# Rouslan/NTracer

Measured on AMD Instinct MI355X. Metric: Mrays/s (primary+shadow), 6-D hypercube @1920x1080, higher is better.
Workload: dtype f32

## Files before the change

ntracer_amd/csrc/nt_box.hpp:

```cpp
#pragma once
#include <type_traits>
#include "nt_pixel.hpp"
#include "nt_box_span.hpp"

namespace {

__device__ __forceinline__ bool box_may_hit(int n, const float *dots, float sx, float sy, float sq) {
    const float osq = dots[0];
    const float ov = fmaf(-dots[2], sy, fmaf(dots[1], sx, dots[3]));
    const float rad2 = (float)n * (1.0f + NT_FUZZ) * (1.0f + NT_FUZZ) * 1.001f;
#ifdef NT_EXP_SKIP_SLABS
    return false;
#else
    return !((osq - rad2) * sq > ov * ov * 1.0001f);
#endif
}

__device__ __forceinline__ void box_background(float in, float &r, float &g, float &b) {
    if (in > 0.0f) { r = in; g = in; b = in; }
    else { r = 0.0f; g = -in; b = -in; }
}

template <int N>
__device__ __forceinline__ void box_color(const float (&o)[N], const float (&dir)[N], bool maybe, float &r, float &g, float &b) {
    bool done = false;
    float shade = 0.0f;

    {
        float num[N];
        bool pre[N];
        float aK = 0.0f, bK = 1.0f, oK = 0.0f;
        bool any = false;
#pragma unroll
        for (int i = 0; i < N; ++i) {
            const float di = dir[i];
            const float s = di < 0.0f ? 1.0f : -1.0f;
            num[i] = s - o[i];
            pre[i] = maybe && ((num[i] > 0.0f && di > 0.0f) || (num[i] < 0.0f && di < 0.0f));
            const float a = fabsf(num[i]), bb = fabsf(di);
            if (pre[i] && (!any || a * bK > aK * bb)) { aK = a; bK = bb; oK = o[i]; any = true; }
        }
        const float mu = 1e-4f * (1.0f + fabsf(oK));
        const float aKm = (aK - mu) * (1.0f - 1e-6f);
#pragma unroll
        for (int i = 0; i < N; ++i) {
            const bool tie = pre[i] && !done && !(fabsf(num[i]) * bK < fabsf(dir[i]) * aKm);
            if (__builtin_amdgcn_ballot_w64(tie) != 0ull) {
                const float di = dir[i];
                const float dist = num[i] / di;
                bool ok = tie && dist > 0.0f;
#pragma unroll
                for (int j = 0; j < N; ++j) {
                    if (j != i) {
                        const float p = dir[j] * dist + o[j];
                        ok = ok && !(fabsf(p) > (1.0f + NT_FUZZ));
                    }
                }
                if (ok) {
                    done = true;
                    if (dist >= FLT_MAX) shade = -1.0f;
                    else {
                        const float sine = di * (di < 0.0f ? 1.0f : -1.0f);
                        shade = sine <= 0.0f ? -sine : 0.0f;
                    }
                }
            }
        }
    }
    if (done && shade >= 0.0f) {
        r = shade * 1.0f;
        g = shade * 0.5f;
        b = shade * 0.5f;
    } else {
        box_background(dir[0], r, g, b);
    }
}

#ifndef NT_BOX_INLINE_MAX_N
#define NT_BOX_INLINE_MAX_N 8
#endif
#ifndef NT_BOX_SETS_MAX_N
#define NT_BOX_SETS_MAX_N NT_BOX_INLINE_MAX_N
#endif
template <int N>
__device__ __forceinline__ void box_classify(const float (&o)[N], const float (&v)[N], float m, bool maybe, bool &hit, bool &unclear,
                                             float &x, float (&near)[N], float &tn, float &vK) {
    float tn2 = -INFINITY;
    tn = -INFINITY;
    vK = 0.0f;
    float tnp = -INFINITY, tfp = INFINITY;
    const float m1p = 1.0f + m;
#pragma unroll
    for (int j = 0; j < N; ++j) {
        const float inv = __builtin_amdgcn_rcpf(v[j]);
        const float c0 = -o[j] * inv;
        const float nr = c0 - fabsf(inv);
        near[j] = nr;
        tnp = fmaxf(tnp, fmaf(-fabsf(inv), m1p, c0));
        tfp = fminf(tfp, fmaf(fabsf(inv), m1p, c0));
        const bool later = nr > tn;
        tn2 = __builtin_amdgcn_fmed3f(tn, tn2, nr);
        vK = later ? v[j] : vK;
        tn = fmaxf(tn, nr);
    }
    const bool miss = tnp > tfp || tfp < 0.0f;
    const float c = 1.0f - m;
    float sum = 0.0f;
#pragma unroll
    for (int j = 0; j < N; ++j) sum = sum + fmaxf(fabsf(fmaf(v[j], tn, o[j])), c);
    const bool inside = sum - (float)N * c <= 1.5f * m;
    const bool sole = (tn - tn2) * fabsf(vK) > m;
    const bool front = tn > 1e-3f && tn < 1e30f;
    hit = maybe && !miss && inside && sole && front;
    unclear = maybe && !miss && !hit;
#ifdef NT_EXP_NOUNCLEAR
    unclear = false;
#endif
    x = hit ? vK : v[0];
}

__device__ __forceinline__ float nt_vmax(float a, float b) { float r; asm("v_max_f32 %0, %1, %2" : "=v"(r) : "v"(a), "v"(b)); return r; }
__device__ __forceinline__ float nt_vmin(float a, float b) { float r; asm("v_min_f32 %0, %1, %2" : "=v"(r) : "v"(a), "v"(b)); return r; }
__device__ __forceinline__ float nt_vmax3(float a, float b, float c) { float r; asm("v_max3_f32 %0, %1, %2, %3" : "=v"(r) : "v"(a), "v"(b), "v"(c)); return r; }
__device__ __forceinline__ float nt_vmin3(float a, float b, float c) { float r; asm("v_min3_f32 %0, %1, %2, %3" : "=v"(r) : "v"(a), "v"(b), "v"(c)); return r; }
__device__ __forceinline__ float nt_vmed3(float a, float b, float c) { float r; asm("v_med3_f32 %0, %1, %2, %3" : "=v"(r) : "v"(a), "v"(b), "v"(c)); return r; }
__device__ __forceinline__ float nt_vmax_abs(float a, float b) { float r; asm("v_max_f32 %0, |%1|, %2" : "=v"(r) : "v"(a), "v"(b)); return r; }
__device__ __forceinline__ float nt_vmax3_abs(float a, float b, float c) { float r; asm("v_max3_f32 %0, %1, |%2|, |%3|" : "=v"(r) : "v"(a), "v"(b), "v"(c)); return r; }
__device__ __forceinline__ float nt_vmin_abs(float a, float b) { float r; asm("v_min_f32 %0, |%1|, %2" : "=v"(r) : "v"(a), "v"(b)); return r; }

#ifndef NT_BOX_TIE_SHORTCUT
#define NT_BOX_TIE_SHORTCUT 1
#endif
#ifndef NT_BOX_TIE_SHORTCUT_MIN_N
#define NT_BOX_TIE_SHORTCUT_MIN_N 6
#endif
#ifndef NT_BOX_TIE_SHORTCUT_MAX_N
#define NT_BOX_TIE_SHORTCUT_MAX_N 8
#endif
#ifndef NT_BOX_TIE_SURE_MAX_ORIGIN
#define NT_BOX_TIE_SURE_MAX_ORIGIN 4.5f
#endif
#ifndef NT_BOX_TIE_SHORTCUT_MIN_WAVES
#define NT_BOX_TIE_SHORTCUT_MIN_WAVES 32768
#endif
#define NT_BOX_SETS_SURE 0x01000000u
#ifndef NT_BOX_STRIP_SPAN
#define NT_BOX_STRIP_SPAN 1
#endif
template <int N>
constexpr bool nt_box_tie_shortcut() { return NT_BOX_TIE_SHORTCUT != 0 && N >= NT_BOX_TIE_SHORTCUT_MIN_N && N <= NT_BOX_TIE_SHORTCUT_MAX_N && N <= NT_BOX_SETS_MAX_N; }

#ifndef NT_BOX_CLASSIFY_SETS_MIN_N
#define NT_BOX_CLASSIFY_SETS_MIN_N 6
#endif
#ifndef NT_BOX_CLASSIFY_SETS_MAX_N
#define NT_BOX_CLASSIFY_SETS_MAX_N 7
#endif
template <int N>
__device__ __forceinline__ void box_classify_sets(const float (&o)[N], const float (&v)[N], float m, uint32_t sets, bool &hit, bool &unclear,
                                                  float &x) {
    float tn = -INFINITY, tn2 = -INFINITY, vK = 0.0f;
    float tnp = -INFINITY, tfp = INFINITY;
    const float m1p = 1.0f + m;
#pragma unroll
    for (int j = 0; j < N; ++j) {
        if (((sets >> (10 + j)) & 1u) != 0u) {
            const float inv = __builtin_amdgcn_rcpf(v[j]);
            const float c0 = -o[j] * inv;
            tfp = nt_vmin(tfp, fmaf(fabsf(inv), m1p, c0));
            if (((sets >> j) & 1u) != 0u) {
                const float nr = c0 - fabsf(inv);
                tnp = nt_vmax(tnp, fmaf(-fabsf(inv), m1p, c0));
                const bool later = nr > tn;
                tn2 = nt_vmed3(tn, tn2, nr);
                vK = later ? v[j] : vK;
                tn = nt_vmax(tn, nr);
            }
        }
    }
    const bool miss = tnp > tfp || tfp < 0.0f;
    const float c = 1.0f - m;
    float sum = 0.0f;
#ifndef NT_EXP_SETS_MASKS
    asm volatile("" : "+s"(sets));
#endif
#pragma unroll
    for (int j = 0; j < N; ++j) {
        if (((sets >> (10 + j)) & 1u) != 0u) {
            asm volatile("" : "+v"(sum));
            sum = sum + nt_vmax_abs(fmaf(v[j], tn, o[j]), c);
        }
    }
    const bool inside = sum - (float)__builtin_popcount((sets >> 10) & 0x3ffu) * c <= 1.5f * m;
    const bool sole = (tn - tn2) * fabsf(vK) > m;
    const bool front = tn > 1e-3f && tn < 1e30f;
    hit = !miss && inside && sole && front;
    unclear = !miss && !hit;
    x = hit ? vK : v[0];
}

template <int N>
__device__ __forceinline__ void box_entries(const float (&o)[N], const float (&v)[N], float (&near)[N], float &tn, float &vK) {
    tn = -INFINITY;
    vK = 0.0f;
#pragma unroll
    for (int j = 0; j < N; ++j) {
        const float inv = __builtin_amdgcn_rcpf(v[j]);
        const float nr = fmaf(-o[j], inv, -fabsf(inv));
        near[j] = nr;
        vK = nr > tn ? v[j] : vK;
        tn = fmaxf(tn, nr);
    }
}

template <int N>
__device__ __forceinline__ void box_resolve(const float (&o)[N], const float (&v)[N], float len, float m, const float (&near)[N], float tn,
                                            float vK, bool unclear, bool &hit, float &x) {
    const float aK = fabsf(vK);
    const float slack = m * __builtin_amdgcn_rcpf(aK), lim = 1.0f - 0.5f * m;
    bool inT[N], inC[N];
    float d[N];
    uint32_t anyC = 0u;
#pragma unroll
    for (int j = 0; j < N; ++j) {
        const bool early = (tn - near[j]) * aK > m;
        const bool robust = fmaf(fabsf(v[j]), slack, fabsf(fmaf(v[j], tn, o[j]))) <= lim;
        inT[j] = unclear && !early;
        inC[j] = unclear && !(robust && early);
        d[j] = 0.0f;
        if (__builtin_amdgcn_ballot_w64(inC[j]) != 0ull) {
            d[j] = v[j] / len;
            anyC |= 1u << j;
        }
    }
    bool done = false, found = false;
    float xs = v[0];
#pragma unroll
    for (int i = 0; i < N; ++i) {
        const bool cand = inT[i] && !done;
        if (__builtin_amdgcn_ballot_w64(cand) != 0ull) {
            const float di = d[i];
            const float dist = ((di < 0.0f ? 1.0f : -1.0f) - o[i]) / di;
            bool ok = cand && di != 0.0f && dist > 0.0f;
#pragma unroll
            for (int j = 0; j < N; ++j) {
                if (j != i && ((anyC >> j) & 1u) != 0u) {
                    const float p = d[j] * dist + o[j];
                    ok = ok && !(inC[j] && fabsf(p) > (1.0f + NT_FUZZ));
                }
            }
            if (ok) {
                done = true;
                if (!(dist >= FLT_MAX)) { found = true; xs = v[i]; }
            }
        }
    }
    if (unclear) {
        hit = found;
        x = xs;
    }
}

typedef __attribute__((address_space(1))) uint8_t *nt_gptr;
__device__ __forceinline__ nt_gptr uniform_ptr(uint8_t *p) {
    const unsigned long long v = reinterpret_cast<unsigned long long>(p);
    const uint32_t lo = (uint32_t)__builtin_amdgcn_readfirstlane((int)(uint32_t)v), hi = (uint32_t)__builtin_amdgcn_readfirstlane((int)(uint32_t)(v >> 32));
    return (nt_gptr)(((unsigned long long)hi << 32) | lo);
}
#define NT_G32(p) (*(__attribute__((address_space(1))) uint32_t *)(p))

template <typename P>
__device__ __forceinline__ void emit_f32x3_at(const NtTarget &tg, P p, float r, float gb) {
    r = r > 0.0f ? r : 0.0f;
    r = r < 1.0f ? r : 1.0f;
    gb = gb > 0.0f ? gb : 0.0f;
    gb = gb < 1.0f ? gb : 1.0f;
    uint32_t vr = __float_as_uint(r), vgb = __float_as_uint(gb);
    uint3 w;
    if (tg.plain_f32[0] == 0 && tg.plain_f32[1] == 1 && tg.plain_f32[2] == 2 && !tg.reversed) {
        w.x = bswap32(vr);
        w.y = bswap32(vgb);
        w.z = w.y;
    } else {
        if (!tg.reversed) { vr = bswap32(vr); vgb = bswap32(vgb); }
        w.x = tg.plain_f32[tg.reversed ? 2 : 0] == 0 ? vr : vgb;
        w.y = tg.plain_f32[1] == 0 ? vr : vgb;
        w.z = tg.plain_f32[tg.reversed ? 0 : 2] == 0 ? vr : vgb;
    }
    if constexpr (std::is_same<P, nt_gptr>::value) {
        typedef uint32_t u32x3 __attribute__((ext_vector_type(3)));
        u32x3 v;
        v.x = w.x; v.y = w.y; v.z = w.z;
        *(__attribute__((address_space(1))) u32x3 *)(p) = v;
    } else {
        *reinterpret_cast<uint3 *>(p) = w;
    }
}
__device__ __forceinline__ void emit_f32x3(const NtTarget &tg, long long offset, float r, float gb) { emit_f32x3_at(tg, tg.dest + offset, r, gb); }

__device__ __forceinline__ float sqrt_in_range(float x) {
    const float s = __builtin_amdgcn_sqrtf(x);
    const float s_dn = __uint_as_float(__float_as_uint(s) - 1u), s_up = __uint_as_float(__float_as_uint(s) + 1u);
    const float vp = fmaf(-s_dn, s, x), vs = fmaf(-s_up, s, x);
    float r = vp <= 0.0f ? s_dn : s;
    r = vs > 0.0f ? s_up : r;
    return r;
}
__device__ __forceinline__ float sqrt_wave(float x) {
    if (__builtin_amdgcn_ballot_w64(!(x >= 0x1p-96f && x < 0x1p96f)) == 0ull) return sqrt_in_range(x);
    return sqrtf(x);
}

template <int N, bool PLAIN, bool DEFER = false, bool REDO = false, bool F32 = false, bool TIE = false>
__device__ __forceinline__ bool box_pixel(const NtTarget &tg, const PixelRef &pr, const float (&org)[N], float (&dir)[N], float sq,
                                          const float (&dots)[4], float sx, float sy, float margin, bool rowhit = true, int face = -1,
                                          uint32_t sets = 0u, bool noclass = false) {
    constexpr bool INL = (F32 || PLAIN) && !REDO && !DEFER;
    const bool redo = REDO || (INL && noclass);
    const bool maybe = redo || (rowhit && (DEFER || INL || box_may_hit(N, dots, sx, sy, sq)));
    float r, g, b;
    bool hit = false, unclear = false;
    float x = dir[0];
#ifndef NT_EXP_NOCLASSIFY
    float near[N], tn = 0.0f, vK = 0.0f;
    constexpr bool CSETS = INL && N >= NT_BOX_CLASSIFY_SETS_MIN_N && N <= NT_BOX_CLASSIFY_SETS_MAX_N;
    auto exact_on_sets = [&]() {
        const float len = sqrt_wave(sq);
        float d[N];
#pragma unroll
        for (int j = 0; j < N; ++j) {
            d[j] = 0.0f;
            if ((sets >> (10 + j)) & 1u) d[j] = dir[j] / len;
        }
        bool done = false;
        x = dir[0];
#pragma unroll
        for (int i = 0; i < N; ++i) {
// ... 307 lines not shown
    }
    if (!(tlo > thi)) {
        code = 15u;
#pragma unroll
        for (int j = 0; j < N; ++j) {
            const float nr = ((vc[j] < 0.0f ? 1.0f : -1.0f) - org[j]) * __builtin_amdgcn_rcpf(vc[j]);
            tn2 = nt_vmed3(tn, tn2, nr);
            const bool later = nr > tn;
            vK = later ? vc[j] : vK;
            gK = later ? g[j] : gK;
            oK = later ? org[j] : oK;
            K = later ? j : K;
            tn = nt_vmax(tn, nr);
        }
        const float vKa = vK - gK, vKb = vK + gK;
        if (K < 13 && vKa * vKb > 0.0f) {
            const float num = (vK < 0.0f ? 1.0f : -1.0f) - oK;
            const float t1 = num * __builtin_amdgcn_rcpf(vKa), t2 = num * __builtin_amdgcn_rcpf(vKb);
            const float t_lo = nt_vmin(t1, t2) * (1.0f - 1e-6f), t_hi = nt_vmax(t1, t2) * (1.0f + 1e-6f);
            const float rK = m * __builtin_amdgcn_rcpf(fabsf(vK) - gK) * (1.0f + 1e-6f);
            bool ok = t_lo > 1e-3f && t_hi < 1e30f;
#pragma unroll
            for (int j = 0; j < N; ++j) {
                const float va = vc[j] - g[j], vb = vc[j] + g[j];
                const float pmax = org[j] + nt_vmax(vb * t_lo, vb * t_hi);
                const float pmin = org[j] + nt_vmin(va * t_lo, va * t_hi);
                const float lim = (1.0f - m - 1e-4f) - (fabsf(vc[j]) + g[j]) * rK;
                ok = ok && (j == K || (pmax <= lim && pmin >= -lim));
            }
            if (ok) code = (uint32_t)K + 1u;
        }
        if (code == 15u && !((tn - tn2) * fabsf(vK) > m)) code = 14u;
        if (code >= 14u) {
            if (sets != nullptr && N <= 10) {
                auto range = [&](int j, float &A, float &B, float &vabs) {
                    const float va = vc[j] - g[j], vb = vc[j] + g[j];
                    const float num = (vc[j] < 0.0f ? 1.0f : -1.0f) - org[j];
                    const float e1 = num * __builtin_amdgcn_rcpf(va), e2 = num * __builtin_amdgcn_rcpf(vb);
                    const float lo = nt_vmin(e1, e2), hi = nt_vmax(e1, e2);
                    const bool same = va * vb > 0.0f;
                    A = same ? lo - fabsf(lo) * 1e-6f : -INFINITY;
                    B = same ? hi + fabsf(hi) * 1e-6f : INFINITY;
                    vabs = same ? fabsf(vc[j]) - g[j] : 0.0f;
                };
                float rA[N], rB[N], rV[N];
                float TN = -INFINITY, TH = -INFINITY;
#pragma unroll
                for (int j = 0; j < N; ++j) {
                    range(j, rA[j], rB[j], rV[j]);
                    TN = nt_vmax(TN, rA[j]);
                    TH = nt_vmax(TH, rB[j]);
                }
                float vmin = INFINITY;
#pragma unroll
                for (int j = 0; j < N; ++j) vmin = rB[j] >= TN ? nt_vmin(vmin, rV[j]) : vmin;
                const float M = m * __builtin_amdgcn_rcpf(vmin) * (1.0f + 1e-5f);
                uint32_t T = 0u, C = 0u;
                float t_lo = INFINITY;
                const float t_hi = TH;
#pragma unroll
                for (int j = 0; j < N; ++j) {
                    const bool inT = rB[j] >= TN - M;
                    T |= inT ? 1u << j : 0u;
                    t_lo = inT ? nt_vmin(t_lo, rA[j]) : t_lo;
                }
#pragma unroll
                for (int j = 0; j < N; ++j) {
                    const float va = vc[j] - g[j], vb = vc[j] + g[j];
                    const float pmax = org[j] + nt_vmax(vb * t_lo, vb * t_hi);
                    const float pmin = org[j] + nt_vmin(va * t_lo, va * t_hi);
                    const float lim = 1.0f - m - 1e-4f;
                    const bool inC = ((T >> j) & 1u) != 0u || !(pmax <= lim && pmin >= -lim);
                    C |= inC ? 1u << j : 0u;
                }
                const bool valid = vmin > 0.0f && t_lo > 1e-3f && t_hi < 1e30f;
                *sets = valid ? (0x80000000u | (C << 10) | T) : 0u;
                if constexpr (SURE) {
                    float wmax = 0.0f;
                    uint32_t far_axes = 0u;
#pragma unroll
                    for (int j = 0; j < N; ++j) {
                        wmax = nt_vmax3_abs(wmax, vc[j] - g[j], vc[j] + g[j]);
                        far_axes |= (__float_as_uint(org[j]) & 0x7fffffffu) > __float_as_uint(NT_BOX_TIE_SURE_MAX_ORIGIN) ? 1u << j : 0u;
                    }
                    const bool sure = valid && C == T && (T & far_axes) == 0u && (t_hi - t_lo) * wmax <= 1.0f;
                    *sets |= sure ? NT_BOX_SETS_SURE : 0u;
                }
            }
        }
    }
    return (unsigned long long)code | ((unsigned long long)sets_value << 32);
}
template <int N>
__device__ __forceinline__ uint32_t box_stretch_code(const float (&org)[N], const float (&right)[N], const float (&up)[N], const float (&fwd)[N],
                                                     const NtTarget &tg, int y, int col) {
    return (uint32_t)box_stretch_code2<N, false>(org, right, up, fwd, tg, y, col);
}

template <int N>
__global__ __launch_bounds__(256) void box_cull_kernel(NtCameraFixed cam, NtTarget tg, uint32_t *out, int ncols) {
    float org[N], right[N], up[N], fwd[N];
    load_camera<N>(cam, org, right, up, fwd);
    const int word = (int)blockIdx.x, row = (int)blockIdx.y * 8 + (int)(threadIdx.x >> 5);
    const int col = word * 32 + (int)(threadIdx.x & 31);
    uint32_t code = 0u;
    if (row < tg.row_count && col < ncols) {
        const int orow = tg.row_begin + row;
        const int y = nt_image_row(tg, orow);
        code = box_stretch_code<N>(org, right, up, fwd, tg, y, col);
    }
    uint32_t packed = code << (4 * (threadIdx.x & 7));
    packed |= (uint32_t)__shfl_xor((int)packed, 1, 64);
    packed |= (uint32_t)__shfl_xor((int)packed, 2, 64);
    packed |= (uint32_t)__shfl_xor((int)packed, 4, 64);
    if (row < tg.row_count && (threadIdx.x & 7) == 0) out[((size_t)blockIdx.z * tg.row_count + row) * tg.cull_words + (col >> 3)] = packed;
}

#ifdef NT_EXP_NOSTORE
#define NT_EXP_STORE_IF if (tg.width < 0)
#else
#define NT_EXP_STORE_IF
#endif
#ifndef NT_TILE_OCC
#define NT_TILE_OCC
#endif
#ifndef NT_BOX_PIN_UP
#define NT_BOX_PIN_UP 1
#endif
#ifndef NT_BOX_LEAN_GROUPS_MAX_N
#define NT_BOX_LEAN_GROUPS_MAX_N 20
#endif
__device__ __forceinline__ bool guard_clear(float t) { return fabsf(__builtin_amdgcn_fractf(t) - 0.5f) > fmaf(t, 0x1p-18f, 0x1p-18f); }
__device__ __forceinline__ float lean_quotient(float d, float sy, float uu, float m2bu, float bb) {
    return fabsf(d) * __builtin_amdgcn_rsqf(fmaf(sy, fmaf(sy, uu, m2bu), bb));
}
template <int N>
__device__ __forceinline__ void pick_component(uint32_t K, const float (&base)[N], const float (&upv)[N], float &bK, float &uK) {
    bK = base[0];
    uK = upv[0];
#pragma unroll
    for (int j = 1; j < N; ++j) {
        bK = K == (uint32_t)j ? base[j] : bK;
        uK = K == (uint32_t)j ? upv[j] : uK;
    }
}
template <int N>
__device__ __forceinline__ float row_dir(const float (&base)[N], const float (&upv)[N], float sy, float (&dir)[N]) {
#pragma unroll
    for (int j = 0; j < N; ++j) dir[j] = base[j] - upv[j] * sy;
    float sq = dir[0] * dir[0];
#pragma unroll
    for (int j = 1; j < N; ++j) sq = sq + dir[j] * dir[j];
    return sq;
}
#ifndef NT_BOX_PASS_ROWS
#define NT_BOX_PASS_ROWS 64
#endif
__device__ __forceinline__ int nt_low_bit(uint32_t m) { return __builtin_ctz(m); }
__device__ __forceinline__ int nt_low_bit(unsigned long long m) { return __builtin_ctzll(m); }
__device__ __forceinline__ int nt_count_bits(uint32_t m) { return __builtin_popcount(m); }
__device__ __forceinline__ int nt_count_bits(unsigned long long m) { return __builtin_popcountll(m); }
__device__ __forceinline__ void nt_clear_bit(uint32_t &m, int bit) { asm("s_bitset0_b32 %0, %1" : "+s"(m) : "s"(bit)); }
__device__ __forceinline__ void nt_clear_bit(unsigned long long &m, int bit) { asm("s_bitset0_b64 %0, %1" : "+s"(m) : "s"(bit)); }
__device__ __forceinline__ void nt_set_bit(uint32_t &m, int bit) { asm("s_bitset1_b32 %0, %1" : "+s"(m) : "s"(bit)); }
__device__ __forceinline__ void nt_set_bit(unsigned long long &m, int bit) { asm("s_bitset1_b64 %0, %1" : "+s"(m) : "s"(bit)); }
__device__ __forceinline__ void nt_drop_low_bit(uint32_t &m, int) { m &= m - 1u; }
__device__ __forceinline__ void nt_drop_low_bit(unsigned long long &m, int bit) { nt_clear_bit(m, bit); }
template <int N, bool F32, int ROWS, int WAVES, bool TIE = false>
__global__ __launch_bounds__(64 * WAVES) NT_TILE_OCC void box_tile_kernel(NtCameraFixed cam, NtTarget tg) {
    static_assert(!TIE || (!F32 && ROWS == 64 && nt_box_tie_shortcut<N>()), "the short cut: packed RGB, 64 x 1, the dimensions it is built for");
    static_assert(ROWS == 8 || ROWS == 16 || ROWS == 64, "a wave's rows: a qword of sixteen codes in LDS or fewer, or one row a lane");
    static_assert(WAVES >= 1 && WAVES <= 4 && WAVES * ROWS <= 64, "the codes of a tile are the work of one wave, a row per lane");
    static_assert(WAVES == 1 ? ROWS == 64 : ROWS <= 16, "one wave a block renders the 64 rows whose codes it worked out itself");
    constexpr int R = ROWS;
    constexpr bool REG = WAVES == 1;
    constexpr int LDS_N = REG ? 1 : 64;
    __shared__ uint32_t s_code[LDS_N];
    __shared__ unsigned long long s_rows[REG ? 1 : 4];
    constexpr bool ALLIN = F32 || N <= NT_BOX_INLINE_MAX_N;
    constexpr bool SETS_LDS = ALLIN && N <= NT_BOX_SETS_MAX_N;
    constexpr uint32_t SETS_MASK = 0x800fffffu | (TIE ? NT_BOX_SETS_SURE : 0u);
    __shared__ uint32_t s_sets[SETS_LDS ? LDS_N : 1];
    __shared__ int s_abort;
    uint32_t lane_cs = 0u;
    const int tid = (int)threadIdx.x;
    const int lane = tid & 63;
    const int wv = __builtin_amdgcn_readfirstlane(tid >> 6);
#ifdef NT_EXP_TRACE
    const unsigned long long trace_t0 = wall_clock64();
    unsigned trace_rows = 0u;
    unsigned long long trace_t1 = 0ull;
#endif
    const unsigned nframes = gridDim.z - (unsigned)tg.lead_frames;
    unsigned frame = blockIdx.z;
    if (tg.lead_frames > 0) {
        const unsigned cols = gridDim.x, q = cols / 4u;
        const bool middle = blockIdx.x >= q && blockIdx.x < cols - q;
        if (!middle) frame -= (unsigned)tg.lead_frames;
        if (frame >= nframes) return;
    }
    float org[N], right[N], up[N], fwd[N], dir[N];
    load_camera<N>(cam, frame, org, right, up, fwd);
    float margin = fabsf(org[0]);
#pragma unroll
    for (int j = 1; j < N; ++j) margin = fmaxf(margin, fabsf(org[j]));
    margin = NT_BOX_MARGIN * (1.0f + margin);
    float dots[4];
    if (cam.buf) {
        const float *dp = cam.dots + (size_t)frame * 4;
        dots[0] = dp[0]; dots[1] = dp[1]; dots[2] = dp[2]; dots[3] = dp[3];
    } else {
        dots[0] = cam.odots[0]; dots[1] = cam.odots[1]; dots[2] = cam.odots[2]; dots[3] = cam.odots[3];
    }
    const int tile_row0 = (int)blockIdx.y * WAVES * R;
    bool strip_out = false;
    if constexpr (NT_BOX_STRIP_SPAN != 0 && N <= NT_BOX_SPAN_MAX_N) {
      if (cam.span != nullptr) {
        const float *sp = cam.span + (size_t)frame * 2;
        const float span_lo = sp[0], span_hi = sp[1];
        const int x_first = (int)blockIdx.x * 64;
        const int x_last = x_first + 63 < tg.width ? x_first + 63 : tg.width - 1;
        const float sx_a = tg.fovI * ((float)x_first - tg.half_w), sx_b = tg.fovI * ((float)x_last - tg.half_w);
        strip_out = fmaxf(sx_a, sx_b) < span_lo || fminf(sx_a, sx_b) > span_hi;
      }
    }
    if (REG || wv == (int)((blockIdx.x + blockIdx.y + frame) % (unsigned)WAVES)) {
        if (tg.abort_word != nullptr) {
            const bool ab = nt_aborted(tg);
            if constexpr (REG) { if (ab) return; }
            else { if (lane == 0) s_abort = ab ? 1 : 0; }
        }
        uint32_t code = 0u;
        uint32_t row_sets = 0u;
        const int trow = tg.row_il > 0 ? ((int)blockIdx.y * WAVES + lane / R) + tg.row_il * (lane % R) : tile_row0 + lane;
        if (!strip_out && lane < WAVES * R && trow < tg.row_count) {
            const int orow = tg.row_begin + trow;
            const int y = nt_image_row(tg, orow);
            if (y < tg.height) {
                const unsigned long long cs = box_stretch_code2<N, (N <= NT_BOX_SETS_MAX_N), TIE>(org, right, up, fwd, tg, y, (int)blockIdx.x);
                code = (uint32_t)cs;
                row_sets = (uint32_t)(cs >> 32);
            }
        }
        if constexpr (REG) {
            lane_cs = (SETS_LDS ? row_sets & SETS_MASK : 0u) | (code << 20);
        } else {
            if (SETS_LDS) s_sets[lane] = row_sets;
            {
                const unsigned long long m0 = __builtin_amdgcn_ballot_w64(code == 0u), m1 = __builtin_amdgcn_ballot_w64(code >= 1u && code <= 13u),
                                         m2 = __builtin_amdgcn_ballot_w64(code == 15u), m3 = __builtin_amdgcn_ballot_w64(code == 14u);
                if (lane == 0) {
                    s_rows[0] = m0;
                    s_rows[1] = m1;
                    s_rows[2] = m2;
                    s_rows[3] = m3;
                }
            }
            uint32_t packed = code << (4 * (lane & 7));
            packed |= (uint32_t)__shfl_xor((int)packed, 1, 64);
            packed |= (uint32_t)__shfl_xor((int)packed, 2, 64);
            packed |= (uint32_t)__shfl_xor((int)packed, 4, 64);
            if ((lane & 7) == 0) {
                const int grp = lane >> 3;
                const int slot = R == 8 ? 2 * grp : grp;
                s_code[slot] = packed;
                if (R == 8) s_code[slot + 1] = 0u;
            }
        }
    }
    if constexpr (!REG) {
        __syncthreads();
        if (tg.abort_word != nullptr && s_abort != 0) return;
    }
#ifdef NT_EXP_TRACE
    trace_t1 = wall_clock64();
#endif
    constexpr int PASS = R == 64 ? NT_BOX_PASS_ROWS : R;
    static_assert(PASS == R || (R == 64 && PASS == 16), "NT_BOX_PASS_ROWS: 64 or 16");
    typedef typename std::conditional<PASS == 64, unsigned long long, uint32_t>::type mask_t;
    const int wrow0 = tile_row0 + wv * R;
    const int il = tg.row_il;
    const int wfirst = il > 0 ? (int)blockIdx.y * WAVES + wv : wrow0;
    if (wfirst < tg.row_count) {
        typedef uint32_t nt_u32x4 __attribute__((ext_vector_type(4)));
        typedef __attribute__((address_space(4))) const nt_u32x4 *nt_rowtab;
        typedef uint32_t nt_u32x16 __attribute__((ext_vector_type(16), aligned(16)));
        typedef __attribute__((address_space(4))) const nt_u32x16 *nt_rowtab4;
        constexpr bool GROUPS = !F32 && N <= NT_BOX_LEAN_GROUPS_MAX_N;
        uint8_t *const frame_base = tg.dest + (long long)frame * tg.frame_stride;
#define NT_ROW_LOAD(rr)                     \
        const nt_u32x4 row_e = tab[(rr)];   \
        const float sy = __uint_as_float(row_e.x)
#define NT_ROW_OFF() ((long long)(((unsigned long long)row_e.w << 32) | row_e.z) + (long long)frame * tg.frame_stride)
#define NT_ROW_PTR() uniform_ptr(frame_base + (long long)(((unsigned long long)row_e.w << 32) | row_e.z))
#define NT_GROUP_PTR(k) uniform_ptr(frame_base + (long long)(((unsigned long long)grp_e[4 * (k) + 3] << 32) | grp_e[4 * (k) + 2]))
#define NT_LANE_OFF() ({ asm volatile("" : "+v"(xoff)); xoff; })
#define NT_CLEAR_BIT(mask, bit) nt_clear_bit(mask, bit)
#define NT_SET_BIT(mask, bit) nt_set_bit(mask, bit)
        int x = (int)blockIdx.x * 64 + lane;
        x = x < tg.width ? x : tg.width - 1;
        uint32_t xoff = (uint32_t)x * (uint32_t)tg.bpp;
        const float sx = tg.fovI * ((float)x - tg.half_w);
        float base[N];
#pragma unroll
        for (int j = 0; j < N; ++j) base[j] = fwd[j] + right[j] * sx;
        float upv[N];
#pragma unroll
        for (int j = 0; j < N; ++j) {
            upv[j] = up[j];
            if (NT_BOX_PIN_UP || F32 || j == 0) asm volatile("" : "+v"(upv[j]));
        }
        float bb = 0.0f, bu = 0.0f, uu = 0.0f;
        bool fastsq = true;
        if (!F32) {
#pragma unroll
            for (int j = 0; j < N; ++j) {
                bb = fmaf(base[j], base[j], bb);
                bu = fmaf(base[j], up[j], bu);
                uu = fmaf(up[j], up[j], uu);
            }
            fastsq = __builtin_amdgcn_ballot_w64(!(bu * bu <= bb * uu * 0.0625f)) == 0ull;
        }
        const float maxv = (float)tg.plain_maxval;
        const float inv_maxv2 = 1.0f / (maxv * maxv);
        const float m2bu = (-2.0f * bu) * inv_maxv2;
        bb = bb * inv_maxv2;
        uu = uu * inv_maxv2;
        const uint32_t lane_code = (lane_cs >> 20) & 15u;
        unsigned long long rows_culled, rows_face, rows_rays, rows_tie;
        if constexpr (REG) {
            rows_culled = __builtin_amdgcn_ballot_w64(lane_code == 0u);
            rows_face = __builtin_amdgcn_ballot_w64(lane_code >= 1u && lane_code <= 13u);
            rows_rays = __builtin_amdgcn_ballot_w64(lane_code == 15u);
            rows_tie = __builtin_amdgcn_ballot_w64(lane_code == 14u);
        } else {
            auto rows_of = [&](int k) {
                const unsigned long long m = s_rows[k];
                return (((unsigned long long)(uint32_t)__builtin_amdgcn_readfirstlane((int)(uint32_t)(m >> 32)) << 32) |
                        (uint32_t)__builtin_amdgcn_readfirstlane((int)(uint32_t)m)) >> (wv * R);
            };
            rows_culled = rows_of(0);
            rows_face = rows_of(1);
            rows_rays = rows_of(2);
            rows_tie = rows_of(3);
        }
        const int lrow = il > 0 ? wfirst + il * lane : wrow0 + lane;
        const int ly = nt_image_row(tg, tg.row_begin + lrow);
        const unsigned long long rows_valid = __builtin_amdgcn_ballot_w64(lane < R && lrow < tg.row_count && ly < tg.height);
#pragma unroll 1
        for (int pass = 0; pass < R / PASS; ++pass) {
        const int slot0 = PASS * pass;
        const int row0 = wrow0 + slot0;
        const int hfirst = il > 0 ? wfirst + il * slot0 : row0;
        if (hfirst >= tg.row_count) break;
        mask_t redo_bits = 0u;
        unsigned long long rowcodes = 0ull;
        if constexpr (!REG) {
            rowcodes = ((unsigned long long)(uint32_t)__builtin_amdgcn_readfirstlane((int)s_code[2 * wv + 1]) << 32) |
                       (uint32_t)__builtin_amdgcn_readfirstlane((int)s_code[2 * wv]);
        }
        auto slot_word = [&](int rr) { return (uint32_t)__builtin_amdgcn_readlane((int)lane_cs, slot0 + rr); };
        auto code_of = [&](int rr) {
            if constexpr (REG) return (slot_word(rr) >> 20) & 15u;
            else return (uint32_t)(rowcodes >> (4 * rr)) & 15u;
        };
        auto sets_of = [&](int rr) {
            if constexpr (!SETS_LDS) return 0u;
            else if constexpr (REG) return slot_word(rr) & SETS_MASK;
            else return (uint32_t)__builtin_amdgcn_readfirstlane((int)s_sets[wv * R + rr]);
        };
        auto rows_with_code = [&](uint32_t c) {
            if constexpr (REG) return (mask_t)(__builtin_amdgcn_ballot_w64(lane_code == c) >> slot0);
            else return (mask_t)__builtin_amdgcn_ballot_w64(lane < PASS && ((uint32_t)(rowcodes >> (4 * (lane & 15))) & 15u) == c);
        };
        const mask_t valid = R > PASS ? (mask_t)(rows_valid >> slot0) & (mask_t)((1ull << (PASS & 63)) - 1ull) : (mask_t)rows_valid;
        const nt_rowtab tab = (nt_rowtab)tg.rowtab + (il > 0 ? row0 : tg.row_begin + row0);
        mask_t quick = (mask_t)(rows_culled >> slot0) & valid, inner = (mask_t)(rows_face >> slot0) & valid;
        mask_t todo = (mask_t)((ALLIN ? rows_rays | rows_tie : rows_rays) >> slot0) & valid;
        if (!ALLIN) redo_bits = (mask_t)(rows_tie >> slot0) & valid;
#ifdef NT_EXP_TRACE
        trace_rows += (unsigned)nt_count_bits(quick) | ((unsigned)nt_count_bits(inner) << 8) |
                      ((unsigned)nt_count_bits((mask_t)(rows_rays >> slot0) & valid) << 16) |
                      ((unsigned)nt_count_bits((mask_t)(rows_tie >> slot0) & valid) << 24);
#endif
        if (!F32) {
            if (!fastsq) {
                todo |= quick | inner;
                quick = 0u;
                inner = 0u;
            }
            auto lean_rows = [&](auto sel8) {
            constexpr bool SEL8 = decltype(sel8)::value;
#ifdef NT_EXP_RED_BY_SHIFT
#define NT_RED_OF(q, d0) ((q) & (uint32_t)((int32_t)__float_as_uint(d0) >> 31))
#else
#define NT_RED_OF(q, d0) ((d0) > 0.0f ? (q) : 0u)
#endif
            auto put_quick = [&](nt_gptr out, float t, float d0) {
                if (SEL8) {
                    const uint32_t q = __float_as_uint(t + 8388608.0f);
                    NT_EXP_STORE_IF NT_G32(out) = __builtin_amdgcn_perm(NT_RED_OF(q, d0), q, tg.plain_sel);
                    return;
                }
                uint32_t q = (uint32_t)(t + 0.5f);
                q = q < tg.plain_maxval ? q : tg.plain_maxval;
                const uint32_t w = NT_RED_OF(q, d0) * tg.plain_mul[0] + q * (tg.plain_mul[1] + tg.plain_mul[2]);
                NT_EXP_STORE_IF NT_G32(out) = tg.reversed ? w : bswap32(w);
            };
            auto put_face = [&](nt_gptr out, float t, float th) {
                if (SEL8) {
                    NT_EXP_STORE_IF NT_G32(out) = __builtin_amdgcn_perm(__float_as_uint(t + 8388608.0f), __float_as_uint(th + 8388608.0f), tg.plain_sel);
                    return;
                }
                uint32_t qr = (uint32_t)(t + 0.5f), qgb = (uint32_t)(th + 0.5f);
                qr = qr < tg.plain_maxval ? qr : tg.plain_maxval;
                qgb = qgb < tg.plain_maxval ? qgb : tg.plain_maxval;
                const uint32_t w = qr * tg.plain_mul[0] + qgb * (tg.plain_mul[1] + tg.plain_mul[2]);
                NT_EXP_STORE_IF NT_G32(out) = tg.reversed ? w : bswap32(w);
            };
            auto full_groups = [](mask_t mask) { return mask & (mask >> 1) & (mask >> 2) & (mask >> 3) & (mask_t)(PASS == 64 ? 0x1111111111111111ull : 0x1111ull); };
            auto lean_group = [&](int g, auto row, auto put) {
                const nt_u32x16 grp_e = *(nt_rowtab4)(tab + g);
                float a[4], b[4];
                unsigned long long fail[4];
#pragma unroll
                for (int k = 0; k < 4; ++k) fail[k] = __builtin_amdgcn_ballot_w64(!row(__uint_as_float(grp_e[4 * k]), a[k], b[k]));
                if (__builtin_expect(((fail[0] | fail[1]) | (fail[2] | fail[3])) == 0ull, 1)) {
                    const uint32_t xo = NT_LANE_OFF();
                    put(NT_GROUP_PTR(0) + xo, a[0], b[0]);
                    put(NT_GROUP_PTR(1) + xo, a[1], b[1]);
                    put(NT_GROUP_PTR(2) + xo, a[2], b[2]);
                    put(NT_GROUP_PTR(3) + xo, a[3], b[3]);
                } else {
                    todo |= (mask_t)((fail[0] != 0ull ? 1u : 0u) | (fail[1] != 0ull ? 2u : 0u) | (fail[2] != 0ull ? 4u : 0u) | (fail[3] != 0ull ? 8u : 0u)) << g;
#pragma unroll
                    for (int k = 0; k < 4; ++k) {
                        if (fail[k] == 0ull) {
                            uint32_t xo = xoff;
                            asm volatile("" : "+v"(xo));
                            put(NT_GROUP_PTR(k) + xo, a[k], b[k]);
                        }
                    }
                }
            };
            auto culled_row = [&](float sy, float &t, float &d0) {
#ifdef NT_EXP_RED_BY_SHIFT
                d0 = upv[0] * sy - base[0];
#else
                d0 = base[0] - upv[0] * sy;
#endif
                t = lean_quotient(d0, sy, uu, m2bu, bb);
                return guard_clear(t);
            };
            auto face_row = [&](float bK, float uK, float sy, float &t, float &th) {
                const float dK = bK - uK * sy;
                t = lean_quotient(dK, sy, uu, m2bu, bb);
                th = t * 0.5f;
                return guard_clear(t) && guard_clear(th);
            };
            if (GROUPS) {
                mask_t full = full_groups(quick);
                quick &= ~(full * 15u);
                while (full != 0u) {
                    const int g = nt_low_bit(full);
                    NT_CLEAR_BIT(full, g);
                    lean_group(g, culled_row, put_quick);
                }
            }
            mask_t quick_stored = 0u;
            for (mask_t rest = quick; rest != 0u;) {
                const int rr = nt_low_bit(rest);
                NT_CLEAR_BIT(rest, rr);
                NT_ROW_LOAD(rr);
                float t, d0;
                if (__builtin_expect(__builtin_amdgcn_ballot_w64(!culled_row(sy, t, d0)) == 0ull, 1)) {
                    put_quick(NT_ROW_PTR() + NT_LANE_OFF(), t, d0);
                    NT_SET_BIT(quick_stored, rr);
                }
            }
            todo |= quick & ~quick_stored;
            while (inner != 0u) {
                const uint32_t code0 = code_of(nt_low_bit(inner));
                float bK0, uK0;
                pick_component<N>(code0 - 1u, base, upv, bK0, uK0);
                mask_t same = inner & rows_with_code(code0);
                inner &= ~same;
                if (GROUPS) {
                    mask_t full = full_groups(same);
                    same &= ~(full * 15u);
                    while (full != 0u) {
                        const int g = nt_low_bit(full);
                        NT_CLEAR_BIT(full, g);
                        lean_group(g, [&](float sy, float &t, float &th) { return face_row(bK0, uK0, sy, t, th); }, put_face);
                    }
                }
                mask_t same_stored = 0u;
                for (mask_t rest = same; rest != 0u;) {
                    const int rr = nt_low_bit(rest);
                    NT_CLEAR_BIT(rest, rr);
                    NT_ROW_LOAD(rr);
                    float t, th;
                    if (__builtin_expect(__builtin_amdgcn_ballot_w64(!face_row(bK0, uK0, sy, t, th)) == 0ull, 1)) {
                        put_face(NT_ROW_PTR() + NT_LANE_OFF(), t, th);
                        NT_SET_BIT(same_stored, rr);
                    }
                }
                todo |= same & ~same_stored;
            }
            };
            if (tg.plain_sel != 0u) lean_rows(std::true_type{});
            else lean_rows(std::false_type{});
        } else {
            while (quick != 0u) {
                const int rr = nt_low_bit(quick);
                nt_drop_low_bit(quick, rr);
                NT_ROW_LOAD(rr);
                const float sq = row_dir<N>(base, upv, sy, dir);
                const float in = dir[0] / sqrt_wave(sq);
                float r, gb, b_;
                box_background(in, r, gb, b_);
                emit_f32x3_at(tg, NT_ROW_PTR() + NT_LANE_OFF(), r, gb);
            }
            while (inner != 0u) {
                const uint32_t code0 = code_of(nt_low_bit(inner));
                float bK0, uK0;
                pick_component<N>(code0 - 1u, base, upv, bK0, uK0);
                mask_t same = inner & rows_with_code(code0);
                inner &= ~same;
                while (same != 0u) {
                    const int rr = nt_low_bit(same);
                    nt_drop_low_bit(same, rr);
                    NT_ROW_LOAD(rr);
                    const float sq = row_dir<N>(base, upv, sy, dir);
                    const float xk = bK0 - uK0 * sy;
                    const float shade = fabsf(xk / sqrt_wave(sq));
                    emit_f32x3_at(tg, NT_ROW_PTR() + NT_LANE_OFF(), shade * 1.0f, shade * 0.5f);
                }
            }
        }
        while (todo != 0u) {
            const int rr = nt_low_bit(todo);
            nt_drop_low_bit(todo, rr);
            const int rcode = (int)code_of(rr);
            const bool rowhit = rcode != 0;
            NT_ROW_LOAD(rr);
            PixelRef pr;
            pr.x = x;
            pr.y = 0;
            pr.offset = NT_ROW_OFF() + (long long)xoff;
            pr.hit_index = 0;
            pr.valid = true;
            const float sq = row_dir<N>(base, upv, sy, dir);
            if (ALLIN) {
                box_pixel<N, !F32, false, false, F32, TIE>(tg, pr, org, dir, sq, dots, sx, sy, margin, rowhit, rcode >= 1 && rcode <= 13 ? rcode - 1 : -1,
                                                       sets_of(rr), rcode == 14);
            } else if (!box_pixel<N, true, true, false, false>(tg, pr, org, dir, sq, dots, sx, sy, margin, rowhit, rcode >= 1 && rcode <= 13 ? rcode - 1 : -1)) {
                redo_bits |= (mask_t)1u << rr;
            }
        }
        if (!ALLIN && lane == 0) {
            while (redo_bits != 0u) {
                const int rr = nt_low_bit(redo_bits);
                nt_drop_low_bit(redo_bits, rr);
                const int mrow = il > 0 ? hfirst + il * rr : row0 + rr;
                atomicOr(tg.redo + ((size_t)frame * tg.row_count + mrow) * tg.redo_words + (blockIdx.x >> 5), 1u << (blockIdx.x & 31));
            }
        }
        }
    }
#ifdef NT_EXP_TRACE
    if (lane == 0) {
        unsigned long long *tr = reinterpret_cast<unsigned long long *>(tg.dest + (long long)nframes * tg.frame_stride) +
                                 ((((size_t)frame * gridDim.y + blockIdx.y) * gridDim.x + blockIdx.x) * WAVES + wv) * 4;
        tr[0] = trace_t0;
        tr[1] = wall_clock64();
        tr[2] = (unsigned long long)__builtin_amdgcn_s_getreg(4 | (31 << 11)) | ((unsigned long long)__builtin_amdgcn_s_getreg(20 | (31 << 11)) << 32);
        tr[3] = (unsigned long long)trace_rows | ((trace_t1 - trace_t0) << 32);
    }
#endif
#undef NT_ROW_LOAD
#undef NT_ROW_OFF
#undef NT_ROW_PTR
#undef NT_GROUP_PTR
#undef NT_LANE_OFF
#undef NT_CLEAR_BIT
#undef NT_SET_BIT
#undef NT_RED_OF
}

template <int N>
int launch_box_fixed(const NtLaunchInfo &li, const NtCamera &cam, const NtTarget &tg_in) {
    NtCameraFixed cf;
    cf.buf = cam.buf;
    cf.dots = cam.dots;
    cf.span = cam.buf ? cam.span : nullptr;
    for (int k = 0; k < 4; ++k) cf.odots[k] = cam.odots[k];
    cf.n = N;
    for (int k = 0; k < 4 * N; ++k) cf.inl[k] = cam.inl[k];
    NtTarget tg = tg_in;
    dim3 grid;
    grid_for(tg, 64, tg.colors_out ? 4 : 4 * NT_BOXROWS, li.nframes, grid);
    tg.cull = nullptr;
    tg.redo = nullptr;
    tg.cull_words = 0;
    tg.redo_words = 0;
    const bool fmt_rgb = tg.plain_bits != 0u && tg.plain_bits <= 10u && tg.bpp == 4 && tg.aligned4;
    const bool fmt_f32 = tg.plain_f32[0] >= 0 && tg.bpp == 12 && tg.aligned4;
    if (li.cull_buf && tg.rowtab && !tg.colors_out && (fmt_rgb || fmt_f32) && li.cull_clean) {
        hipStream_t st = (hipStream_t)li.stream;
        NtBoxTileGeom geom;
        geom.rows = li.tile_rows;
        geom.waves = li.tile_waves;
        const bool r64 = geom.rows == 64, r16 = geom.rows == 16;
        const int wpb = geom.waves;
        const int tile_rows = geom.rows * geom.waves;
        dim3 tgrid((unsigned)((tg.width + 63) / 64), (unsigned)((tg.row_count + tile_rows - 1) / tile_rows), (unsigned)li.nframes);
        tg.redo_words = ((tg.width + 63) / 64 + 31) / 32;
        tg.redo = li.cull_buf;
        tg.lead_frames = li.nframes >= 8 ? (li.nframes < 96 ? li.nframes : 96) : 0;
        if (tg.row_il > 0) tg.lead_frames = li.nframes >= 32 ? 16 : 0;
        if ((long long)li.nframes + tg.lead_frames > 65535) tg.lead_frames = 0;
        tgrid.z += (unsigned)tg.lead_frames;
        if (fmt_rgb) {
            bool tie = false;
            if constexpr (nt_box_tie_shortcut<N>()) tie = r64 && (unsigned long long)tgrid.x * tgrid.y * (unsigned)li.nframes >= (unsigned long long)NT_BOX_TIE_SHORTCUT_MIN_WAVES;
            if (tie) {
                if constexpr (nt_box_tie_shortcut<N>()) hipLaunchKernelGGL((box_tile_kernel<N, false, 64, 1, true>), tgrid, dim3(64), 0, st, cf, tg);
            } else if (r64) hipLaunchKernelGGL((box_tile_kernel<N, false, 64, 1>), tgrid, dim3(64), 0, st, cf, tg);
            else if (r16 && wpb == 3) hipLaunchKernelGGL((box_tile_kernel<N, false, 16, 3>), tgrid, dim3(192), 0, st, cf, tg);
            else if (r16) hipLaunchKernelGGL((box_tile_kernel<N, false, 16, 4>), tgrid, dim3(256), 0, st, cf, tg);
            else hipLaunchKernelGGL((box_tile_kernel<N, false, 8, 4>), tgrid, dim3(256), 0, st, cf, tg);
            if constexpr (N > NT_BOX_INLINE_MAX_N) {
                const long long rwords = (long long)tg.row_count * li.nframes * tg.redo_words;
                const int split = rwords < 48 * 1024 ? 2 : 1;
                const int rpb = 4 / split;
                const dim3 rgrid((unsigned)tg.redo_words, (unsigned)((tg.row_count + rpb - 1) / rpb), (unsigned)li.nframes);
                if (split == 2) hipLaunchKernelGGL((box_redo_kernel<N, 2>), rgrid, dim3(256), 0, st, cf, tg);
                else hipLaunchKernelGGL((box_redo_kernel<N, 1>), rgrid, dim3(256), 0, st, cf, tg);
            }
        } else {
            if (r64) hipLaunchKernelGGL((box_tile_kernel<N, true, 64, 1>), tgrid, dim3(64), 0, st, cf, tg);
            else if (r16 && wpb == 3) hipLaunchKernelGGL((box_tile_kernel<N, true, 16, 3>), tgrid, dim3(192), 0, st, cf, tg);
            else if (r16) hipLaunchKernelGGL((box_tile_kernel<N, true, 16, 4>), tgrid, dim3(256), 0, st, cf, tg);
            else hipLaunchKernelGGL((box_tile_kernel<N, true, 8, 4>), tgrid, dim3(256), 0, st, cf, tg);
        }
        return 0;
    }
    if (li.cull_buf && !tg.colors_out) {
        const int ncols = (tg.width + 63) / 64;
        const int words = (ncols + 31) / 32;
        tg.cull_words = 4 * words;
        hipLaunchKernelGGL(box_cull_kernel<N>, dim3((unsigned)words, (unsigned)((tg.row_count + 7) / 8), (unsigned)li.nframes), dim3(256), 0,
                           (hipStream_t)li.stream, cf, tg, li.cull_buf, ncols);
        tg.cull = li.cull_buf;
    }
    hipLaunchKernelGGL(box_kernel<N>, grid, dim3(256), 0, (hipStream_t)li.stream, cf, tg);
    return 0;
}

}
// ... 1 lines not shown
```

Baseline: 1.138 million.

## Add specialized two-axis edge-row fast path with compile-time slab sets

Adds an edge-row path in the tie-shortcut lean pass. Rows where every lane's classification word names exactly two candidate slab axes are grouped by identical word and classified with a 2-D specialization of box_classify_sets. The slab-set mask is a template constant, so the loop unrolls to just those two axes. Rows that classify cleanly are stored directly and removed from the todo set, avoiding the general per-row path. This costs extra code size, register pressure and ballots for grouping.

```diff
diff --git a/ntracer_amd/csrc/nt_box.hpp b/ntracer_amd/csrc/nt_box.hpp
--- a/ntracer_amd/csrc/nt_box.hpp
+++ b/ntracer_amd/csrc/nt_box.hpp
@@ -156,9 +156,10 @@
 #ifndef NT_BOX_CLASSIFY_SETS_MAX_N
 #define NT_BOX_CLASSIFY_SETS_MAX_N 7
 #endif
-template <int N>
+template <int N, uint32_t FIXED = 0u>
 __device__ __forceinline__ void box_classify_sets(const float (&o)[N], const float (&v)[N], float m, uint32_t sets, bool &hit, bool &unclear,
                                                   float &x) {
+    if constexpr (FIXED != 0u) sets = FIXED;
     float tn = -INFINITY, tn2 = -INFINITY, vK = 0.0f;
     float tnp = -INFINITY, tfp = INFINITY;
     const float m1p = 1.0f + m;
@@ -182,7 +183,7 @@
     const float c = 1.0f - m;
     float sum = 0.0f;
 #ifndef NT_EXP_SETS_MASKS
-    asm volatile("" : "+s"(sets));
+    if constexpr (FIXED == 0u) asm volatile("" : "+s"(sets));
 #endif
 #pragma unroll
     for (int j = 0; j < N; ++j) {
@@ -796,6 +797,13 @@
 #pragma unroll
     for (int j = 1; j < N; ++j) sq = sq + dir[j] * dir[j];
     return sq;
+}
+#ifndef NT_BOX_EDGE_ROWS
+#define NT_BOX_EDGE_ROWS 1
+#endif
+template <int N>
+constexpr bool nt_box_edge_rows() {
+    return NT_BOX_EDGE_ROWS != 0 && N >= NT_BOX_CLASSIFY_SETS_MIN_N && N <= NT_BOX_CLASSIFY_SETS_MAX_N && N <= NT_BOX_SETS_MAX_N && N <= NT_BOX_INLINE_MAX_N;
 }
 #ifndef NT_BOX_PASS_ROWS
 #define NT_BOX_PASS_ROWS 64
@@ -931,6 +939,7 @@
         typedef uint32_t nt_u32x16 __attribute__((ext_vector_type(16), aligned(16)));
         typedef __attribute__((address_space(4))) const nt_u32x16 *nt_rowtab4;
         constexpr bool GROUPS = !F32 && N <= NT_BOX_LEAN_GROUPS_MAX_N;
+        constexpr bool EDGE = TIE && !F32 && REG && PASS == 64 && nt_box_edge_rows<N>();
         uint8_t *const frame_base = tg.dest + (long long)frame * tg.frame_stride;
 #define NT_ROW_LOAD(rr)                     \
         const nt_u32x4 row_e = tab[(rr)];   \
@@ -1150,6 +1159,70 @@
                     }
                 }
                 todo |= same & ~same_stored;
+            }
+            if constexpr (EDGE) {
+                mask_t edge = fastsq ? (mask_t)rows_rays & valid : (mask_t)0u;
+                if (edge != 0u) {
+                    const uint32_t lT = lane_cs & 0x3ffu, lC = (lane_cs >> 10) & 0x3ffu;
+                    const bool two = (lane_cs & 0x80000000u) != 0u && (lT & ~lC) == 0u && __builtin_popcount(lC) == 2 && (lT == lC || __builtin_popcount(lT) == 1);
+                    edge &= (mask_t)__builtin_amdgcn_ballot_w64(two);
+                }
+                auto put_edge = [&](nt_gptr out, float t, float tgb, bool red) {
+                    if (SEL8) {
+                        const uint32_t q8r = __float_as_uint(t + 8388608.0f), q8gb = __float_as_uint(tgb + 8388608.0f);
+                        NT_EXP_STORE_IF NT_G32(out) = __builtin_amdgcn_perm(red ? q8r : 0u, q8gb, tg.plain_sel);
+                        return;
+                    }
+                    uint32_t qr = (uint32_t)(t + 0.5f), qgb = (uint32_t)(tgb + 0.5f);
+                    qr = qr < tg.plain_maxval ? qr : tg.plain_maxval;
+                    qgb = qgb < tg.plain_maxval ? qgb : tg.plain_maxval;
+                    const uint32_t w = (red ? qr : 0u) * tg.plain_mul[0] + qgb * (tg.plain_mul[1] + tg.plain_mul[2]);
+                    NT_EXP_STORE_IF NT_G32(out) = tg.reversed ? w : bswap32(w);
+                };
+                mask_t edge_stored = 0u;
+                while (edge != 0u) {
+                    const uint32_t w0 = slot_word(nt_low_bit(edge)) & 0x800fffffu;
+                    const mask_t same = edge & (mask_t)__builtin_amdgcn_ballot_w64((lane_cs & 0x800fffffu) == w0);
+                    edge &= ~same;
+                    const uint32_t c0 = (w0 >> 10) & 0x3ffu;
+                    const uint32_t ja = (uint32_t)__builtin_ctz(c0), jb = 31u - (uint32_t)__builtin_clz(c0);
+                    float bA, uA, bB, uB;
+                    pick_component<N>(ja, base, upv, bA, uA);
+                    pick_component<N>(jb, base, upv, bB, uB);
+                    float oA = org[0], oB = org[0];
+#pragma unroll
+                    for (int j = 1; j < N; ++j) {
+                        oA = ja == (uint32_t)j ? org[j] : oA;
+                        oB = jb == (uint32_t)j ? org[j] : oB;
+                    }
+                    auto set_rows = [&](auto tsel) {
+                        constexpr uint32_t WORD = 0x80000000u | (3u << 10) | decltype(tsel)::value;
+                        for (mask_t rest = same; rest != 0u;) {
+                            const int rr = nt_low_bit(rest);
+                            NT_CLEAR_BIT(rest, rr);
+                            NT_ROW_LOAD(rr);
+                            const float o2[2] = {oA, oB};
+                            const float v2[2] = {bA - uA * sy, bB - uB * sy};
+                            const float v0 = base[0] - upv[0] * sy;
+                            bool hit, unclear;
+                            float x;
+                            box_classify_sets<2, WORD>(o2, v2, margin, WORD, hit, unclear, x);
+                            x = hit ? x : v0;
+                            const float t = lean_quotient(x, sy, uu, m2bu, bb);
+                            const float tgb = hit ? t * 0.5f : t;
+                            const bool ok = ((int)!unclear & (int)guard_clear(t) & (int)guard_clear(tgb)) != 0;
+                            if (__builtin_expect(__builtin_amdgcn_ballot_w64(!ok) == 0ull, 1)) {
+                                put_edge(NT_ROW_PTR() + NT_LANE_OFF(), t, tgb, hit || x > 0.0f);
+                                NT_SET_BIT(edge_stored, rr);
+                            }
+                        }
+                    };
+                    const bool inA = ((w0 >> ja) & 1u) != 0u, inB = ((w0 >> jb) & 1u) != 0u;
+                    if (inA && inB) set_rows(std::integral_constant<uint32_t, 3u>{});
+                    else if (inA) set_rows(std::integral_constant<uint32_t, 1u>{});
+                    else set_rows(std::integral_constant<uint32_t, 2u>{});
+                }
+                todo &= ~edge_stored;
             }
             };
             if (tg.plain_sel != 0u) lean_rows(std::true_type{});
```

New measurement: 1.157 million, median of 6. 1.7% higher.
